# ZLkanyo009/Yolo-compression-and-deployment-in-FPGA

Hardware: AMD Instinct MI355X
Metric: images/sec slim_yolo_v2 int8 416x416 (higher is better)
Workload: dtype int8; 1 GPU; slim_yolo_v2_q_bf int8, batch 64 per GPU, 416x416, 2 classes, conf 0.01; global_batch=64, parallelism=batch-shard x1, streams_per_gpu=4, ring_workgroups_per_launch=128, input=f32, input_batches_rotated=4

## Files before the change

### yolo-compression-and-deployment-in-fpga_amd/csrc/convpx.hip

```cpp
#include "y355_fp32epi.h"
#include "y355_rowring.h"
#include <cstring>
#include <type_traits>
#ifndef PX_R31
#define PX_R31 11
#define PX_R41 6
#endif
#ifndef PX_DIAG
#define PX_DIAG 0
#endif

namespace {
using namespace y355dev;

template <int CIN, int NTN, int NCB, bool POOL>
struct PxGeom {
    static constexpr int PXB = CIN;
    static constexpr int KPP = CIN >= 64 ? CIN / 64 : 1;
    static constexpr int KS = CIN >= 64 ? 9 * KPP : 5;
    static constexpr int CPB = 16 * NTN;
    static constexpr int COUT = CPB * NCB;
    static constexpr int NFRAG = NCB * KS * NTN;
    static_assert(CIN == 32 || CIN == 64 || CIN == 128, "input channels");
    static_assert(!(POOL && CIN < 64), "pooled layers: one tap per k-step");
};
}

template <int CIN, int NTN, int NCB, bool POOL, int NW, int FOLD>
__global__ __launch_bounds__(NW * 64, (NW + 3) / 4) void convpx_kernel(const ConvParams p, const RowRingArgs a) {
    using G = PxGeom<CIN, NTN, NCB, POOL>;
    constexpr int PXB = G::PXB, KPP = G::KPP, KS = G::KS, CPB = G::CPB, COUT = G::COUT;
    constexpr int NPS = NW / NCB;
    constexpr int NV = POOL ? 4 : 1;
    static_assert(NW % NCB == 0, "waves per channel block");
    static_assert(NTN == 4 || NTN == 2, "16- or 8-byte stores");
    extern __shared__ __attribute__((aligned(16))) char smem[];
    const int tid = threadIdx.x;
    const int lane = tid & 63;
    const int wave = __builtin_amdgcn_readfirstlane(tid >> 6);
    const int cb = wave % NCB, ps = wave / NCB;
    const int li = lane & 15, g = lane >> 4;

    v4i wf[KS][NTN];
#pragma unroll
    for (int ks = 0; ks < KS; ++ks)
#pragma unroll
        for (int n = 0; n < NTN; ++n) wf[ks][n] = *(const v4i *)(p.w + ((size_t)(cb * KS + ks) * NTN + n) * 1024 + lane * 16);
    v4i cin[NTN];
    float bf[NTN][4];
#pragma unroll
    for (int n = 0; n < NTN; ++n) {
        const v4i bv = *(const v4i *)(p.bias_t + cb * CPB + 4 * NTN * g + 4 * n);
#pragma unroll
        for (int r = 0; r < 4; ++r) {
            cin[n][r] = FOLD == 2 ? bv[r] + 0x4B400000 : FOLD == 1 ? bv[r] : 0;
            bf[n][r] = (float)bv[r];
        }
    }
    const Requant rq = p.rq;
    const float s_pos = __int_as_float(__builtin_amdgcn_readfirstlane(__float_as_int(ldexpf(1.0f, rq.lk - rq.sh))));
    const float s_neg = __int_as_float(__builtin_amdgcn_readfirstlane(__float_as_int((float)rq.neg_mul * ldexpf(1.0f, -rq.sh))));
    const float c_pos = FOLD == 2 ? MAGIC - MAGIC * s_pos : MAGIC, c_neg = FOLD == 2 ? MAGIC - MAGIC * s_neg : MAGIC;
    float spv = s_pos, snv = s_neg, cpv = c_pos, cnv = c_neg;
    asm volatile("" : "+v"(spv), "+v"(snv), "+v"(cpv), "+v"(cnv));
    const float scl = ldexpf(1.0f, rq.shl);

    using Ring = RowRing<PXB, NW, POOL>;
    int gbeg, gend;
    if (!Ring::share(a, gbeg, gend)) return;
    const Ring ring(a, p.in, smem, p.H, p.W, lane, wave, gend);
    constexpr int MUL = Ring::MUL;
    const int H = ring.H, Ho = ring.Ho, Wo = ring.Wo, npw = ring.npw, rowb = ring.rowb, RM = ring.RM;

    int nstamp = 0;
    auto stamp = [&]() {
#if PX_DIAG
#if PX_DIAG == 2
        if (p.stamps && lane == 0 && nstamp < 16 && blockIdx.x < 128) p.stamps[((size_t)blockIdx.x * NW + wave) * 16 + nstamp++] = __builtin_amdgcn_s_memrealtime();
#else
        if (p.stamps && tid == 0 && nstamp < 32) p.stamps[(size_t)blockIdx.x * 32 + nstamp++] = __builtin_amdgcn_s_memrealtime();
#endif
#endif
    };
    (void)nstamp;
    stamp();
    RowChunk ch = ring.chunk_at(gbeg);
    ring.issue_rows(ch.lo, ch.hi);
    int loaded = ch.hi;
    unsigned int nsat = 0;
    int gg = gbeg, nstores = -1;
    for (;;) {
        stamp();
        wait_vmcnt_upto<16>(nstores);
        asm volatile("s_waitcnt lgkmcnt(0)" ::: "memory");
        stamp();
        __builtin_amdgcn_s_barrier();
        ring.late_rows(ch, loaded);
        stamp();
        const int gnext = gg + (ch.g1 - ch.g0);
        const bool more = gnext < gend;
        RowChunk nx = ch;
        if (more) nx = ring.chunk_at(gnext);
        int pf_r0, pf_nr;
        ring.next_window(ch, nx, more, loaded, pf_r0, pf_nr);
        int pfc = ring.rr0;
        auto prefetch = [&](int count) {
            if (ring.issue_pieces(pf_r0, pf_nr, pfc, count) > 0) nstores = 0;
        };
        stamp();
        int8_t *outb = p.out + (((size_t)ch.b * (Ho + 2) + 1) * (Wo + 2) + 1) * COUT + cb * CPB;
        const int rbase = ch.b * (H + 2);

        float ymx = MAGIC, ymn = MAGIC;
        auto issue = [&](int grp, v4i (&acc)[NV][NTN]) {
            int oy, ox;
            ring.locate(grp, oy, ox);
            const int ar = rbase + MUL * oy, x0 = MUL * ox;
            constexpr int NC = POOL ? 4 : 3;
            int xoff[NC], roff[NC];
#pragma unroll
            for (int c = 0; c < NC; ++c) {
                xoff[c] = Ring::read_off(x0 + c, CIN == 32 ? 0 : g);
                roff[c] = ((ar + c) & RM) * rowb;
            }
#pragma unroll
            for (int v = 0; v < NV; ++v)
#pragma unroll
                for (int n = 0; n < NTN; ++n) acc[v][n] = cin[n];
            if constexpr (!POOL) {
                v4i bq[KS];
#pragma unroll
                for (int ks = 0; ks < KS; ++ks) {
                    if constexpr (CIN == 32) {
                        const int t0 = 2 * ks, t1 = 2 * ks + 1 < 9 ? 2 * ks + 1 : 8;
                        const int o0 = roff[t0 / 3] + xoff[t0 % 3], o1 = roff[t1 / 3] + xoff[t1 % 3];
                        bq[ks] = *(const v4i *)(smem + (g < 2 ? o0 : o1) + 16 * (g & 1));
                    } else {
                        const int tap = ks / KPP, h = ks % KPP;
                        bq[ks] = *(const v4i *)(smem + roff[tap / 3] + (xoff[tap % 3] ^ (h << 6)));
                    }
                }
#pragma unroll
                for (int ks = 0; ks < KS; ++ks)
#pragma unroll
                    for (int n = 0; n < NTN; ++n) acc[0][n] = __builtin_amdgcn_mfma_i32_16x16x64_i8(wf[ks][n], bq[ks], acc[0][n], 0, 0, 0);
                __builtin_amdgcn_sched_group_barrier(0x100, KS, 0);
                __builtin_amdgcn_sched_group_barrier(0x008, KS * NTN, 0);
            } else {
                v4i bq[4][4][KPP];
                auto rd = [&](int r) {
#pragma unroll
                    for (int c = 0; c < 4; ++c)
#pragma unroll
                        for (int h = 0; h < KPP; ++h) bq[r][c][h] = *(const v4i *)(smem + roff[r] + (xoff[c] ^ (h << 6)));
                };
                auto mm = [&](int r) {
#pragma unroll
                    for (int dy = 0; dy < 2; ++dy) {
                        const int ty = r - dy;
                        if (ty < 0 || ty > 2) continue;
#pragma unroll
                        for (int c = 0; c < 4; ++c)
#pragma unroll
                            for (int dx = 0; dx < 2; ++dx) {
                                const int tx = c - dx;
                                if (tx < 0 || tx > 2) continue;
#pragma unroll
                                for (int h = 0; h < KPP; ++h)
#pragma unroll
                                    for (int n = 0; n < NTN; ++n)
                                        acc[2 * dy + dx][n] = __builtin_amdgcn_mfma_i32_16x16x64_i8(wf[(ty * 3 + tx) * KPP + h][n], bq[r][c][h],
                                                                                                   acc[2 * dy + dx][n], 0, 0, 0);
                            }
                    }
                };
                if constexpr (KPP == 1) {
                    rd(0);
                    rd(1);
                    mm(0);
                    rd(2);
                    mm(1);
                    rd(3);
                    mm(2);
                    mm(3);
                    constexpr int RDS = 4 * KPP, M03 = 6 * KPP * NTN, M12 = 12 * KPP * NTN;
                    __builtin_amdgcn_sched_group_barrier(0x100, 2 * RDS, 0);
                    __builtin_amdgcn_sched_group_barrier(0x008, M03, 0);
                    __builtin_amdgcn_sched_group_barrier(0x100, RDS, 0);
                    __builtin_amdgcn_sched_group_barrier(0x008, M12, 0);
                    __builtin_amdgcn_sched_group_barrier(0x100, RDS, 0);
                    __builtin_amdgcn_sched_group_barrier(0x008, M12 + M03, 0);
                } else {
#pragma unroll
                    for (int r = 0; r < 4; ++r) {
                        rd(r);
                        mm(r);
                    }
                }
            }
        };
        auto finish = [&](int grp, const v4i (&acc)[NV][NTN], auto coldc) {
            constexpr bool COLD = decltype(coldc)::value;
            int oy, ox;
            ring.locate(grp, oy, ox);
            unsigned int word[NTN];
#pragma unroll
            for (int n = 0; n < NTN; ++n) {
                float pos[4], neg[4];
#pragma unroll
                for (int r = 0; r < 4; ++r) {
                    int m = acc[0][n][r];
                    if constexpr (POOL) m = max(max(m, acc[1][n][r]), max(acc[2][n][r], acc[3][n][r]));
                    const float tf = FOLD == 2 ? __int_as_float(m) : FOLD == 1 ? (float)m : fmaf((float)m, scl, bf[n][r]);
                    pos[r] = fmaf(tf, spv, cpv);
                    neg[r] = fmaf(tf, snv, cnv);
                }
                if constexpr (!COLD) word[n] = epi_word_hot<false>(pos, neg, ymx, ymn);
                else {
                    float yc[4];
#pragma unroll
                    for (int r = 0; r < 4; ++r) {
                        const float y = vmax(pos[r], neg[r]);
                        yc[r] = __builtin_amdgcn_fmed3f(y, QLO, QHI);
                        nsat += (grp * 16 + li < npw && y != yc[r]) ? 1u : 0u;
                    }
                    word[n] = pack4(yc[0], yc[1], yc[2], yc[3]);
                }
            }
            int8_t *dst = outb + ((oy * (Wo + 2) + ox) * COUT + 4 * NTN * g);
            if constexpr (NTN == 4) *(v4i *)dst = (v4i){(int)word[0], (int)word[1], (int)word[2], (int)word[3]};
            else *(uint2 *)dst = make_uint2(word[0], word[NTN - 1]);
        };
        nstores = 0;
        {
            v4i acc[NV][NTN];
#pragma unroll 1
            for (int grp = ch.g0 + ps; grp < ch.g1; grp += NPS) {
                issue(grp, acc);
                prefetch(a.ppg);
                finish(grp, acc, std::false_type{});
                ++nstores;
            }
            prefetch(1 << 30);
        }
        if (__builtin_amdgcn_ballot_w64(ymx > QHI || ymn < QLO) != 0ull) {
            v4i accC[NV][NTN];
#pragma unroll 1
            for (int grp = ch.g0 + ps; grp < ch.g1; grp += NPS) {
                issue(grp, accC);
                finish(grp, accC, std::true_type{});
            }
            nstores = -1;
        }
        stamp();
        if (!more) break;
        gg = gnext;
        ch = nx;
    }
    asm volatile("s_waitcnt vmcnt(0)" ::: "memory");
    stamp();
    if (nsat) atomicAdd(&p.ctr->sat, (unsigned long long)nsat);
}

namespace {
template <int CIN, int NTN, int NCB, bool POOL>
void px_pack(const int8_t *q_w, int cout, int8_t *dst) {
    using G = PxGeom<CIN, NTN, NCB, POOL>;
    memset(dst, 0, (size_t)G::NFRAG * 1024);
    for (int cb = 0; cb < NCB; ++cb)
        for (int ks = 0; ks < G::KS; ++ks)
            for (int n = 0; n < NTN; ++n)
                for (int l = 0; l < 64; ++l) {
                    const int i = l & 15, g = l >> 4;
                    const int ch = cb * G::CPB + 4 * NTN * (i >> 2) + 4 * n + (i & 3);
                    const int tap = CIN == 32 ? 2 * ks + (g >> 1) : ks / G::KPP;
                    const int c0 = CIN == 32 ? 16 * (g & 1) : 64 * (ks % G::KPP) + 16 * g;
                    if (tap > 8 || ch >= cout) continue;
                    for (int kk = 0; kk < 16; ++kk)
                        dst[(((size_t)cb * G::KS + ks) * NTN + n) * 1024 + l * 16 + kk] = q_w[((size_t)ch * CIN + c0 + kk) * 9 + tap];
                }
}

template <int CIN, int NTN, int NCB, bool POOL, int NW>
struct PxInst {
    using G = PxGeom<CIN, NTN, NCB, POOL>;
    static constexpr int NPS = NW / NCB;
    template <int FOLD>
    static void launch_(const ConvParams &p_in, const RowRingArgs &a, size_t lds, hipStream_t s) {
        ConvParams p = p_in;
        p.ev_start = p.ev_stop = nullptr;
        int grid = y355_cu_count();
        if (p_in.grid_limit > 0 && p_in.grid_limit < grid) grid = p_in.grid_limit;
        if (grid > a.total_groups) grid = a.total_groups;
        Y355_LAUNCH((convpx_kernel<CIN, NTN, NCB, POOL, NW, FOLD>), dim3(grid), dim3(NW * 64), lds, s, p_in.ev_start, p_in.ev_stop, p, a);
    }
    static bool launch(const ConvParams &p, int rounds, hipStream_t s) {
        if (p.cstride != G::COUT || !p.out_halo || p.W < 16 || (POOL && ((p.H | p.W) & 1))) return false;
        if ((long long)p.B * (p.H + 2) * (p.W + 2) * G::PXB >= (1ll << 31)) return false;
        const RowRingArgs a = rowring_args<G::PXB, NW, NPS, POOL>(p.B, p.H, p.W, rounds);
        const size_t lds = rowring_lds_bytes<G::PXB>(a);
        if (lds > 160 * 1024) return false;
        const int fold = y355_fp32_fold(p.rq);
        if (fold == 2) launch_<2>(p, a, lds, s);
        else if (fold == 1) launch_<1>(p, a, lds, s);
        else launch_<0>(p, a, lds, s);
        return true;
    }
    static int prepare() {
        int e = (int)hipFuncSetAttribute((const void *)convpx_kernel<CIN, NTN, NCB, POOL, NW, 0>, hipFuncAttributeMaxDynamicSharedMemorySize, 160 * 1024);
        if (!e) e = (int)hipFuncSetAttribute((const void *)convpx_kernel<CIN, NTN, NCB, POOL, NW, 1>, hipFuncAttributeMaxDynamicSharedMemorySize, 160 * 1024);
        if (!e) e = (int)hipFuncSetAttribute((const void *)convpx_kernel<CIN, NTN, NCB, POOL, NW, 2>, hipFuncAttributeMaxDynamicSharedMemorySize, 160 * 1024);
        return e;
    }
};
using PX_C3_1 = PxInst<32, 4, 1, false, 8>;
using PX_C3_2 = PxInst<64, 2, 2, true, 8>;
using PX_C4_1 = PxInst<64, 4, 2, false, 8>;
using PX_C4_2 = PxInst<128, 2, 4, true, 8>;
}

int y355_prepare_conv_px(void) {
    int e = PX_C3_1::prepare();
    if (!e) e = PX_C3_2::prepare();
    if (!e) e = PX_C4_1::prepare();
    if (!e) e = PX_C4_2::prepare();
    return e;
}

size_t y355_px_packed_bytes(int kid) {
    switch (kid) {
    case Y355_K_CONV3_1: return (size_t)PX_C3_1::G::NFRAG * 1024;
    case Y355_K_CONV3_2: return (size_t)PX_C3_2::G::NFRAG * 1024;
    case Y355_K_CONV4_1: return (size_t)PX_C4_1::G::NFRAG * 1024;
    case Y355_K_CONV4_2: return (size_t)PX_C4_2::G::NFRAG * 1024;
    default: return 0;
    }
}

bool y355_pack_px(int kid, const int8_t *q_w, int cout, int cin, int8_t *dst) {
    switch (kid) {
    case Y355_K_CONV3_1: if (cin != 32 || cout != 64) return false; px_pack<32, 4, 1, false>(q_w, cout, dst); return true;
    case Y355_K_CONV3_2: if (cin != 64 || cout != 64) return false; px_pack<64, 2, 2, true>(q_w, cout, dst); return true;
    case Y355_K_CONV4_1: if (cin != 64 || cout != 128) return false; px_pack<64, 4, 2, false>(q_w, cout, dst); return true;
    case Y355_K_CONV4_2: if (cin != 128 || cout != 128) return false; px_pack<128, 2, 4, true>(q_w, cout, dst); return true;
    default: return false;
    }
}

bool y355_launch_conv_px(int kid, const ConvParams &p, hipStream_t s) {
    if ((p.mode & 0xff) != 0 || p.guard || !y355_fp32_exact(p.rq) || !y355_fp32_slope_ok(p.rq)) return false;
    switch (kid) {
    case Y355_K_CONV3_1: return PX_C3_1::launch(p, PX_R31, s);
    case Y355_K_CONV3_2: return PX_C3_2::launch(p, 2, s);
    case Y355_K_CONV4_1: return PX_C4_1::launch(p, PX_R41, s);
    case Y355_K_CONV4_2: return PX_C4_2::launch(p, 2, s);
    default: return false;
    }
}
```

### yolo-compression-and-deployment-in-fpga_amd/csrc/y355_rowring.h

```cpp
#pragma once
#include "y355_dev.h"

namespace y355dev {
struct RowRingArgs {
    int total_groups;
    int ngi;
    int cg;
    int pwl;
    int logr;
    int ppg;
};
struct RowChunk { int b, g0, g1, lo, hi; };

template <int PXB, int NW, int NPS, bool POOL>
inline RowRingArgs rowring_args(int B, int H, int W, int rounds) {
    constexpr int PPP = 1024 / PXB;
    RowRingArgs a;
    const int Ho = POOL ? H / 2 : H, Wo = POOL ? W / 2 : W;
    a.ngi = (Ho * Wo + 15) / 16;
    a.total_groups = a.ngi * B;
    a.cg = rounds * NPS;
    a.pwl = (W + 2 + PPP - 1) / PPP * PPP;
    const int rows2 = (2 * 16 * a.cg + Wo - 1) / Wo + 1;
    const int need = (POOL ? 2 : 1) * rows2 + 2;
    a.logr = 2;
    while ((1 << a.logr) < need) ++a.logr;
    const int newrows = (POOL ? 2 : 1) * ((16 * a.cg + Wo - 1) / Wo + 1);
    const int ppr = a.pwl / PPP, rs = ppr < NW ? NW / ppr : 1, cpw = ppr < NW ? 1 : (ppr + NW - 1) / NW;
    const int per_wave = (newrows + rs - 1) / rs * cpw;
    a.ppg = (per_wave + rounds - 1) / rounds;
    return a;
}
template <int PXB>
inline size_t rowring_lds_bytes(const RowRingArgs &a) { return ((size_t)a.pwl * PXB) << a.logr; }

template <int PXB, int NW, bool POOL>
struct RowRing {
    static constexpr int PPP = 1024 / PXB;
    static constexpr int CPX = PXB / 16;
    static constexpr int MUL = POOL ? 2 : 1;
    const RowRingArgs a;
    const char *const in;
    char *const smem;
    int H, PW, Ho, Wo, npw, rowb;
    float invWo;
    int gend;
    int R, RM;
    int li, dpx, dch, ppr, RS, CPW, pc0, rr0, goff0;

    __device__ __forceinline__ static bool share(const RowRingArgs &a, int &gbeg, int &gend) {
        const int G_ = gridDim.x;
        gbeg = (int)((long long)a.total_groups * blockIdx.x / G_), gend = (int)((long long)a.total_groups * (blockIdx.x + 1) / G_);
        return gbeg < gend;
    }
    __device__ __forceinline__ RowRing(const RowRingArgs &a_, const void *in_, char *smem_, int H_, int W, int lane, int wave, int gend_)
        : a(a_), in((const char *)in_), smem(smem_), gend(gend_) {
        H = H_;
        PW = W + 2;
        const int PWL = a.pwl;
        Ho = POOL ? H >> 1 : H, Wo = POOL ? W >> 1 : W;
        npw = Ho * Wo;
        rowb = PWL * PXB;
        invWo = 1.0f / (float)Wo;
        R = 1 << a.logr, RM = R - 1;
        li = lane & 15;
        dpx = lane / CPX, dch = lane % CPX;
        ppr = PWL / PPP;
        RS = ppr < NW ? NW / ppr : 1;
        CPW = ppr < NW ? 1 : (ppr + NW - 1) / NW;
        pc0 = ppr < NW ? wave % ppr : wave;
        rr0 = ppr < NW ? (wave / ppr < RS ? wave / ppr : (1 << 28)) : 0;
        goff0 = lane_off(pc0);
    }
    __device__ __forceinline__ RowChunk chunk_at(int gg) const {
        RowChunk c;
        c.b = gg / a.ngi;
        c.g0 = gg - c.b * a.ngi;
        c.g1 = min(min(c.g0 + a.cg, a.ngi), c.g0 + (gend - gg));
        const int ya = (16 * c.g0) / Wo, yb = (min(16 * c.g1, npw) - 1) / Wo;
        c.lo = c.b * (H + 2) + MUL * ya;
        c.hi = c.b * (H + 2) + MUL * yb + (POOL ? 4 : 3);
        return c;
    }
    __device__ __forceinline__ int lane_off(int pc) const {
        const int col = pc * PPP + dpx;
        int sch = dch;
        if constexpr (CPX == 4) sch ^= ((col >> 2) & 1) << 1;
        if constexpr (CPX == 8) sch ^= ((col >> 1) & 3) << 1;
        return min(col, PW - 1) * PXB + 16 * sch;
    }
    __device__ __forceinline__ static int read_off(int x, int sch) {
        if constexpr (CPX == 4) sch ^= ((x >> 2) & 1) << 1;
        if constexpr (CPX == 8) sch ^= ((x >> 1) & 3) << 1;
        return x * PXB + 16 * sch;
    }
    __device__ __forceinline__ int issue_pieces(int r0, int nrows, int &rr, int count) const {
        int done = 0;
        for (; rr < nrows && done < count; rr += RS) {
            const int row = r0 + rr;
            const char *src = in + (size_t)row * (size_t)(PW * PXB);
            char *dst = smem + (row & RM) * rowb;
            glds16(src + goff0, dst + pc0 * 1024);
            ++done;
            for (int j = 1; j < CPW; ++j) {
                const int pc = pc0 + j * NW;
                if (pc < ppr) {
                    glds16(src + lane_off(pc), dst + pc * 1024);
                    ++done;
                }
            }
        }
        return done;
    }
    __device__ __forceinline__ void issue_rows(int r0, int r1) const {
        int rr = rr0;
        issue_pieces(r0, r1 - r0, rr, 1 << 30);
    }
    __device__ __forceinline__ void late_rows(const RowChunk &ch, int &loaded) const {
        if (loaded < ch.hi) {
            issue_rows(max(loaded, ch.lo), ch.hi);
            loaded = ch.hi;
            asm volatile("s_waitcnt vmcnt(0)" ::: "memory");
            __builtin_amdgcn_s_barrier();
        }
    }
    __device__ __forceinline__ void next_window(const RowChunk &ch, const RowChunk &nx, bool more, int &loaded, int &r0, int &nr) const {
        r0 = 0, nr = 0;
        if (more) {
            const int top = min(nx.hi, ch.lo + R);
            r0 = max(loaded, nx.lo);
            if (top > r0) {
                nr = top - r0;
                loaded = top;
            }
        }
    }
    __device__ __forceinline__ void locate(int grp, int &oy, int &ox) const {
        const int pc = min(grp * 16 + li, npw - 1);
        oy = (int)(((float)pc + 0.5f) * invWo);
        ox = pc - oy * Wo;
    }
};
}
```

Before: 338,300 images/sec.

## Use non-power-of-two LDS row ring for pooled conv layers and raise rounds

Replaces the power-of-two LDS row ring with a modular ring sized to fill the LDS budget for pooled layers. Row offsets use a rebased modulo with a single conditional subtract instead of a mask. Rounds for the conv3_2 and conv4_2 layers rise from 2 to 3, and the host shrinks rounds when there are too few groups per CU. The aim is more rows per chunk and deeper prefetch, which cuts barriers and reloads, at the cost of extra offset arithmetic and possible load imbalance.

```diff
diff --git a/yolo-compression-and-deployment-in-fpga_amd/csrc/convpx.hip b/yolo-compression-and-deployment-in-fpga_amd/csrc/convpx.hip
--- a/yolo-compression-and-deployment-in-fpga_amd/csrc/convpx.hip
+++ b/yolo-compression-and-deployment-in-fpga_amd/csrc/convpx.hip
@@ -5,6 +5,16 @@
 #ifndef PX_R31
 #define PX_R31 11
 #define PX_R41 6
+#endif
+#ifndef PX_R32
+#define PX_R32 3
+#define PX_R42 3
+#endif
+#ifndef PX_RMIN
+#define PX_RMIN 2
+#endif
+#ifndef PX_MODR
+#define PX_MODR(pool) (pool)
 #endif
 #ifndef PX_DIAG
 #define PX_DIAG 0
@@ -65,12 +75,12 @@
     asm volatile("" : "+v"(spv), "+v"(snv), "+v"(cpv), "+v"(cnv));
     const float scl = ldexpf(1.0f, rq.shl);
 
-    using Ring = RowRing<PXB, NW, POOL>;
+    using Ring = RowRing<PXB, NW, POOL, PX_MODR(POOL)>;
     int gbeg, gend;
     if (!Ring::share(a, gbeg, gend)) return;
-    const Ring ring(a, p.in, smem, p.H, p.W, lane, wave, gend);
+    Ring ring(a, p.in, smem, p.H, p.W, lane, wave, gend);
     constexpr int MUL = Ring::MUL;
-    const int H = ring.H, Ho = ring.Ho, Wo = ring.Wo, npw = ring.npw, rowb = ring.rowb, RM = ring.RM;
+    const int H = ring.H, Ho = ring.Ho, Wo = ring.Wo, npw = ring.npw;
 
     int nstamp = 0;
     auto stamp = [&]() {
@@ -85,6 +95,7 @@
     (void)nstamp;
     stamp();
     RowChunk ch = ring.chunk_at(gbeg);
+    ring.rebase(ch.lo, true);
     ring.issue_rows(ch.lo, ch.hi);
     int loaded = ch.hi;
     unsigned int nsat = 0;
@@ -121,7 +132,7 @@
 #pragma unroll
             for (int c = 0; c < NC; ++c) {
                 xoff[c] = Ring::read_off(x0 + c, CIN == 32 ? 0 : g);
-                roff[c] = ((ar + c) & RM) * rowb;
+                roff[c] = ring.row_off(ar + c);
             }
 #pragma unroll
             for (int v = 0; v < NV; ++v)
@@ -256,6 +267,7 @@
         if (!more) break;
         gg = gnext;
         ch = nx;
+        ring.rebase(ch.lo);
     }
     asm volatile("s_waitcnt vmcnt(0)" ::: "memory");
     stamp();
@@ -285,21 +297,29 @@
 struct PxInst {
     using G = PxGeom<CIN, NTN, NCB, POOL>;
     static constexpr int NPS = NW / NCB;
+    static int grid_for(const ConvParams &p_in, const RowRingArgs &a) {
+        int grid = y355_cu_count();
+        if (p_in.grid_limit > 0 && p_in.grid_limit < grid) grid = p_in.grid_limit;
+        if (grid > a.total_groups) grid = a.total_groups;
+        return grid;
+    }
     template <int FOLD>
     static void launch_(const ConvParams &p_in, const RowRingArgs &a, size_t lds, hipStream_t s) {
         ConvParams p = p_in;
         p.ev_start = p.ev_stop = nullptr;
-        int grid = y355_cu_count();
-        if (p_in.grid_limit > 0 && p_in.grid_limit < grid) grid = p_in.grid_limit;
-        if (grid > a.total_groups) grid = a.total_groups;
+        const int grid = grid_for(p_in, a);
         Y355_LAUNCH((convpx_kernel<CIN, NTN, NCB, POOL, NW, FOLD>), dim3(grid), dim3(NW * 64), lds, s, p_in.ev_start, p_in.ev_stop, p, a);
     }
     static bool launch(const ConvParams &p, int rounds, hipStream_t s) {
         if (p.cstride != G::COUT || !p.out_halo || p.W < 16 || (POOL && ((p.H | p.W) & 1))) return false;
         if ((long long)p.B * (p.H + 2) * (p.W + 2) * G::PXB >= (1ll << 31)) return false;
-        const RowRingArgs a = rowring_args<G::PXB, NW, NPS, POOL>(p.B, p.H, p.W, rounds);
+        RowRingArgs a = rowring_args<G::PXB, NW, NPS, POOL, PX_MODR(POOL)>(p.B, p.H, p.W, rounds);
+        if constexpr (PX_MODR(POOL)) {
+            int r = a.cg / NPS;
+            while (r > PX_RMIN && a.total_groups < 3 * a.cg * grid_for(p, a)) a = rowring_args<G::PXB, NW, NPS, POOL, true>(p.B, p.H, p.W, --r);
+        }
         const size_t lds = rowring_lds_bytes<G::PXB>(a);
-        if (lds > 160 * 1024) return false;
+        if (lds > ROWRING_LDS_MAX) return false;
         const int fold = y355_fp32_fold(p.rq);
         if (fold == 2) launch_<2>(p, a, lds, s);
         else if (fold == 1) launch_<1>(p, a, lds, s);
@@ -351,9 +371,9 @@
     if ((p.mode & 0xff) != 0 || p.guard || !y355_fp32_exact(p.rq) || !y355_fp32_slope_ok(p.rq)) return false;
     switch (kid) {
     case Y355_K_CONV3_1: return PX_C3_1::launch(p, PX_R31, s);
-    case Y355_K_CONV3_2: return PX_C3_2::launch(p, 2, s);
+    case Y355_K_CONV3_2: return PX_C3_2::launch(p, PX_R32, s);
     case Y355_K_CONV4_1: return PX_C4_1::launch(p, PX_R41, s);
-    case Y355_K_CONV4_2: return PX_C4_2::launch(p, 2, s);
+    case Y355_K_CONV4_2: return PX_C4_2::launch(p, PX_R42, s);
     default: return false;
     }
 }
diff --git a/yolo-compression-and-deployment-in-fpga_amd/csrc/y355_rowring.h b/yolo-compression-and-deployment-in-fpga_amd/csrc/y355_rowring.h
--- a/yolo-compression-and-deployment-in-fpga_amd/csrc/y355_rowring.h
+++ b/yolo-compression-and-deployment-in-fpga_amd/csrc/y355_rowring.h
@@ -7,24 +7,30 @@
     int ngi;
     int cg;
     int pwl;
-    int logr;
+    int nrows;
     int ppg;
 };
 struct RowChunk { int b, g0, g1, lo, hi; };
 
-template <int PXB, int NW, int NPS, bool POOL>
+constexpr size_t ROWRING_LDS_MAX = 160 * 1024;
+template <int PXB, int NW, int NPS, bool POOL, bool MODR = false>
 inline RowRingArgs rowring_args(int B, int H, int W, int rounds) {
     constexpr int PPP = 1024 / PXB;
     RowRingArgs a;
     const int Ho = POOL ? H / 2 : H, Wo = POOL ? W / 2 : W;
     a.ngi = (Ho * Wo + 15) / 16;
     a.total_groups = a.ngi * B;
+    a.pwl = (W + 2 + PPP - 1) / PPP * PPP;
+    const auto need_rows = [&](int r) { return (POOL ? 2 : 1) * ((2 * 16 * r * NPS + Wo - 1) / Wo + 1) + 2; };
+    if constexpr (MODR) {
+        const int fit = (int)(ROWRING_LDS_MAX / ((size_t)a.pwl * PXB));
+        while (rounds > 1 && need_rows(rounds) > fit) --rounds;
+        a.nrows = need_rows(rounds) > fit ? need_rows(rounds) : fit;
+    } else {
+        a.nrows = 4;
+        while (a.nrows < need_rows(rounds)) a.nrows *= 2;
+    }
     a.cg = rounds * NPS;
-    a.pwl = (W + 2 + PPP - 1) / PPP * PPP;
-    const int rows2 = (2 * 16 * a.cg + Wo - 1) / Wo + 1;
-    const int need = (POOL ? 2 : 1) * rows2 + 2;
-    a.logr = 2;
-    while ((1 << a.logr) < need) ++a.logr;
     const int newrows = (POOL ? 2 : 1) * ((16 * a.cg + Wo - 1) / Wo + 1);
     const int ppr = a.pwl / PPP, rs = ppr < NW ? NW / ppr : 1, cpw = ppr < NW ? 1 : (ppr + NW - 1) / NW;
     const int per_wave = (newrows + rs - 1) / rs * cpw;
@@ -32,9 +38,9 @@
     return a;
 }
 template <int PXB>
-inline size_t rowring_lds_bytes(const RowRingArgs &a) { return ((size_t)a.pwl * PXB) << a.logr; }
+inline size_t rowring_lds_bytes(const RowRingArgs &a) { return (size_t)a.pwl * PXB * a.nrows; }
 
-template <int PXB, int NW, bool POOL>
+template <int PXB, int NW, bool POOL, bool MODR = false>
 struct RowRing {
     static constexpr int PPP = 1024 / PXB;
     static constexpr int CPX = PXB / 16;
@@ -46,6 +52,7 @@
     float invWo;
     int gend;
     int R, RM;
+    int brow = 0, bofs = 0;
     int li, dpx, dch, ppr, RS, CPW, pc0, rr0, goff0;
 
     __device__ __forceinline__ static bool share(const RowRingArgs &a, int &gbeg, int &gend) {
@@ -62,7 +69,7 @@
         npw = Ho * Wo;
         rowb = PWL * PXB;
         invWo = 1.0f / (float)Wo;
-        R = 1 << a.logr, RM = R - 1;
+        R = a.nrows, RM = R - 1;
         li = lane & 15;
         dpx = lane / CPX, dch = lane % CPX;
         ppr = PWL / PPP;
@@ -71,6 +78,20 @@
         pc0 = ppr < NW ? wave % ppr : wave;
         rr0 = ppr < NW ? (wave / ppr < RS ? wave / ppr : (1 << 28)) : 0;
         goff0 = lane_off(pc0);
+    }
+    __device__ __forceinline__ void rebase(int lo, bool first = false) {
+        if constexpr (MODR) {
+            int s = first ? 0 : bofs + lo;
+            s = s >= R ? s - R : s;
+            brow = lo, bofs = s - lo;
+        }
+    }
+    __device__ __forceinline__ int row_off(int row) const {
+        if constexpr (MODR) {
+            const unsigned int s = (unsigned int)(row + bofs);
+            return (int)min(s, s - (unsigned int)R) * rowb;
+        } else
+            return (row & RM) * rowb;
     }
     __device__ __forceinline__ RowChunk chunk_at(int gg) const {
         RowChunk c;
@@ -99,7 +120,7 @@
         for (; rr < nrows && done < count; rr += RS) {
             const int row = r0 + rr;
             const char *src = in + (size_t)row * (size_t)(PW * PXB);
-            char *dst = smem + (row & RM) * rowb;
+            char *dst = smem + row_off(row);
             glds16(src + goff0, dst + pc0 * 1024);
             ++done;
             for (int j = 1; j < CPW; ++j) {
```

New measurement: 338,600 images/sec, median of 2. No clear change (+0.1%).
